# fatlipp/eacham

Measured on AMD Instinct MI355X. Metric: image-pairs matched/s + BA iters/s, 200-frame/50k-landmark synthetic, higher is better.
Workload: dtype i8; 1 GPU; S200 matching: 200 frames x 2000 kpts x 256-D, 19900 unordered pairs (both directions + mutual check); pairs_per_rank=19900, parallelism=pairs sharded over 1 GPU(s)

## Files before the change

eacham_amd/csrc/match_screen.hpp:

```cpp
#pragma once

#include <cmath>
#include <cstdint>

#if defined(__HIPCC__)
#define EACHAM_SCREEN_HD __host__ __device__
#else
#define EACHAM_SCREEN_HD
#endif

namespace eacham {
namespace screen {

constexpr int CENTRE = 64;
constexpr int STEP = 4;
constexpr int MAX_D2 = 256 * 255 * 255;
constexpr int MAX_M = 60;

EACHAM_SCREEN_HD inline int mag_value(int c) { return c < 16 ? c : (c < 24 ? 16 + 2 * (c - 16) : 32 + 4 * (c - 24)); }
EACHAM_SCREEN_HD inline int decode(int code) {
    const int m = mag_value(code & 31);
    return (code & 32) ? -m : m;
}
EACHAM_SCREEN_HD inline int encode(int x) {
    const int y = x - CENTRE;
    const int a = y < 0 ? -y : y;
    int c;
    if (a < 64) c = (a + 1) >> 2;
    else if (a < 128) c = 16 + ((a - 64 + 3) >> 3);
    else c = 24 + ((a - 128 + 7) >> 4);
    return (y < 0 && c != 0) ? (c | 32) : c;
}
EACHAM_SCREEN_HD inline int reconstruct(int code) { return CENTRE + STEP * decode(code); }

EACHAM_SCREEN_HD inline void pack32(const unsigned char* codes, uint32_t out[6]) {
    for (int w = 0; w < 6; ++w) out[w] = 0u;
    for (int e = 0; e < 32; ++e) {
        const int bit = 6 * e, w = bit >> 5, sh = bit & 31;
        const uint32_t v = codes[e] & 63u;
        out[w] |= v << sh;
        if (sh > 26) out[w + 1] |= v >> (32 - sh);
    }
}
EACHAM_SCREEN_HD inline int unpack32(const uint32_t in[6], int e) {
    const int bit = 6 * e, w = bit >> 5, sh = bit & 31;
    uint32_t v = in[w] >> sh;
    if (sh > 26) v |= in[w + 1] << (32 - sh);
    return (int)(v & 63u);
}

constexpr int STEP_BYTES = 1536, HI_PLANE = 1024, TILE_ROWS = 32;
struct FragSrc { int row, ks, h; };
EACHAM_SCREEN_HD constexpr FragSrc frag16_src(int u, int S, int lane) { return FragSrc{16 * u + (lane & 15), 2 * S + (lane >> 5), (lane >> 4) & 1}; }
EACHAM_SCREEN_HD constexpr int query16_tile(int s4) { return s4 >> 1; }
EACHAM_SCREEN_HD constexpr FragSrc query16_src(int s4, int S, int lane) { return frag16_src(s4 & 1, S, lane); }
EACHAM_SCREEN_HD constexpr int frag_lo_offset(FragSrc f) { return f.ks * STEP_BYTES + 16 * (f.row + TILE_ROWS * f.h); }
EACHAM_SCREEN_HD constexpr int frag_hi_offset(FragSrc f) { return f.ks * STEP_BYTES + HI_PLANE + 8 * (f.row + TILE_ROWS * f.h); }
EACHAM_SCREEN_HD constexpr int frag_kblock(FragSrc f) { return 2 * f.ks + f.h; }
EACHAM_SCREEN_HD constexpr int acc16_row(int u, int lane, int r) { return 16 * u + 4 * (lane >> 4) + r; }
EACHAM_SCREEN_HD constexpr bool frag16_separable() {
    for (int u = 0; u < 2; ++u)
        for (int S = 0; S < 2; ++S)
            for (int l = 0; l < 64; ++l) {
                if (frag_lo_offset(frag16_src(u, S, l)) != frag_lo_offset(frag16_src(0, 0, l)) + frag_lo_offset(frag16_src(u, S, 0))) return false;
                if (frag_hi_offset(frag16_src(u, S, l)) != frag_hi_offset(frag16_src(0, 0, l)) + frag_hi_offset(frag16_src(u, S, 0)) - HI_PLANE) return false;
            }
    return true;
}
static_assert(frag16_separable(), "lane offset + fragment offset");

EACHAM_SCREEN_HD inline double slack(int s_a, int e_b) { return sqrt((double)s_a) + sqrt((double)e_b); }

EACHAM_SCREEN_HD inline int lower_d2(unsigned n1, int s_a, int e_b) {
    const double l = (double)STEP * sqrt((double)n1) - slack(s_a, e_b);
    if (!(l > 0.0)) return 0;
    const double f = floor(l * l) - 1.0;
    return f <= 0.0 ? 0 : (f >= (double)MAX_D2 ? MAX_D2 : (int)f);
}
EACHAM_SCREEN_HD inline int upper_d2(unsigned u, int s_a, int e_b) {
    const double h = (double)STEP * sqrt((double)u) + slack(s_a, e_b);
    const double c = ceil(h * h) + 1.0;
    return c >= (double)MAX_D2 ? MAX_D2 : (int)c;
}

}
}
```

eacham_amd/csrc/matcher.hip:

```cpp
#include "context.hpp"
#include "match_plan.hpp"
#include "match_screen.hpp"
#include "match_tail.hpp"

#include <algorithm>
#include <climits>
#include <cstdlib>
#include <type_traits>

namespace eacham {

typedef int v4i __attribute__((ext_vector_type(4)));
typedef int v16i __attribute__((ext_vector_type(16)));
typedef const v4i __attribute__((address_space(1)))* gfrag_t;
typedef const int __attribute__((address_space(1)))* gint_t;

constexpr int PADH = 8350000;
constexpr int KEY_SHIFT = 7;
constexpr int KEY_MASK = (1 << KEY_SHIFT) - 1;
constexpr int CHUNK_TILES = 1 << KEY_SHIFT;
constexpr int MAX_ROWS = 16384;
constexpr int WG_THREADS = 256;
constexpr int WAVES = WG_THREADS / 64;
constexpr int MATCH_NSUB = 2;
// ... 690 lines not shown
    uint4* rr = rowres + (size_t)p * row_stride + ROWS_WAVE * wb;
#pragma unroll
    for (int s = 0; s < NSUB; ++s) {
        const int gi = ROWS_WAVE * wave + 32 * s + cl;
        const uint2 gc = GATHER ? pk[gi < item.y ? gi : 0] : make_uint2(0u, 0u);
        const int ca = GATHER ? ((gint_t)frames[pairs[gc.x].x].norm)[gc.y] : Aca[ROWS_WAVE * wb + 32 * s + cl];
        int cls1[2] = {e1[s], x1[s]}, cls2[2] = {e2[s], x2[s]}, clst[2] = {et[s], xt[s]};
        unsigned v1 = 0xffffffffu, v2 = 0xffffffffu, t1 = 0;
#pragma unroll
        for (int c = 0; c < 2; ++c) {
            const int o1 = __shfl_xor(cls1[c], 32), o2 = __shfl_xor(cls2[c], 32), ot = __shfl_xor(clst[c], 32);
            const int tt = o1 < cls1[c] ? ot : (o1 == cls1[c] ? imin(ot, clst[c]) : clst[c]);
            int m1 = cls1[c], m2 = cls2[c];
            top2_merge(m1, m2, o1, o2);
            const unsigned w1 = m1 == BIG ? 0xffffffffu : (unsigned)(2 * (m1 + ca) + c);
            const unsigned w2 = m2 == BIG ? 0xffffffffu : (unsigned)(2 * (m2 + ca) + c);
            t1 = w1 < v1 ? (unsigned)tt : t1;
            v2 = umin(umin(umax(v1, w1), v2), w2);
            v1 = umin(v1, w1);
        }
        if constexpr (GATHER) {
            if (h == 0 && gi < item.y) rowres[(size_t)gc.x * row_stride + gc.y] = make_uint4(v1, t1, v2, 0);
        } else {
            if (h == 0) rr[32 * s + cl] = make_uint4(v1, t1, v2, 0);
        }
    }
}

typedef int v2i __attribute__((ext_vector_type(2)));
typedef int v6i __attribute__((ext_vector_type(6)));
typedef int v8i __attribute__((ext_vector_type(8)));
typedef float v4f __attribute__((ext_vector_type(4)));
__device__ __forceinline__ void lds_read_frag64(v2i& dst, unsigned addr, int offset_bytes) {
    asm volatile("ds_read_b64 %0, %1 offset:%2" : "=v"(dst) : "v"(addr), "n"(offset_bytes));
}
__device__ __forceinline__ float fmin3(float a, float b, float c) {
    float d;
    asm("v_min3_f32 %0, %1, %2, %3" : "=v"(d) : "v"(a), "v"(b), "v"(c));
    return d;
}
template <int METRIC>
__device__ __forceinline__ bool ratio_pass(int d2_best, int d2_second, double ratio);
struct OpenList {
    const int* seghead;
    int* segcount;
    uint2* cands;
    int2* items;
    int* n_items;
};
struct ScreenFrag { v4i lo; v2i hi; };
__device__ __forceinline__ v8i screen_operand(const ScreenFrag& f) { return v8i{f.lo[0], f.lo[1], f.lo[2], f.lo[3], f.hi[0], f.hi[1], 0, 0}; }

template <int METRIC>
__global__ __launch_bounds__(WG_THREADS, 3) void match_screen_kernel(const FrameDev* __restrict__ frames, const int2* __restrict__ pairs,
                                                                     int wgs_per_pair, uint4* __restrict__ rowres, int row_stride, double ratio,
                                                                     unsigned long long* __restrict__ openmask, int mask_stride,
                                                                     OpenList ol) {
    constexpr int NSUB = 2;
    constexpr int NQ = 4, NU = 2, NS = 2;
    constexpr int KS = NU * NS;
    static_assert(KS == SCREEN_KS && 2 * NS == SCREEN_KS && screen::STEP_BYTES == SCREEN_STEP_BYTES, "match_screen.hpp maps this stored tile");
    constexpr int TILE_V4 = SCREEN_TILE_BYTES / 16;
    constexpr int ROWS_WAVE = 32 * NSUB, ROWS_WG = WAVES * ROWS_WAVE;
    constexpr float BIGF = 3.0e38f;
    constexpr int SCALE = (int)0x82828282u;
    constexpr int NT = SCREEN_CALL_TILES, RING = 3 * NT;
    static_assert(NT == 2 && KS == 4 && NT * 32 == 64, "the waits of a call are counted for two tiles of four steps; wave 0 carries the constants of a call");
    __shared__ v4i sB[RING][TILE_V4];
    __shared__ __attribute__((aligned(16))) float sHb[RING][32];
    const int tid = threadIdx.x;
    const int lane = tid & 63;
    const int wave = __builtin_amdgcn_readfirstlane(tid >> 6);
    const int rb = blockIdx.x % wgs_per_pair;
    const int p = blockIdx.x / wgs_per_pair;
    const int2 pr = pairs[p];
    const FrameDev A = frames[pr.x], B = frames[pr.y];
    const int A_even = ((gint_t)A.meta)[0], A_tiles = ((gint_t)A.meta)[1];
    const int T = ((gint_t)B.meta)[2];
    if (rb * (ROWS_WG / 32) >= A_tiles) return;
    const int wb = rb * WAVES + wave;
    const bool active = NSUB * wb < A_tiles;
    typedef const __attribute__((address_space(1))) char* gbytes_t;
    typedef const float __attribute__((address_space(1)))* gfloat_t;
    const gbytes_t Aimg = (gbytes_t)A.screen, Bimg = (gbytes_t)B.screen;
    const gfloat_t Am2 = (gfloat_t)(Aimg + (size_t)A.ntiles * SCREEN_TILE_BYTES), Bm2 = (gfloat_t)(Bimg + (size_t)B.ntiles * SCREEN_TILE_BYTES);
    const int wbc = active ? wb : 0;

    v6i a[NQ][NS];
#pragma unroll
    for (int s = 0; s < NQ; ++s)
#pragma unroll
        for (int S = 0; S < NS; ++S) {
            const screen::FragSrc src = screen::query16_src(s, S, lane);
            const gbytes_t tb = Aimg + (size_t)(NSUB * wbc + screen::query16_tile(s)) * SCREEN_TILE_BYTES;
            const v4i lo = *(const v4i __attribute__((address_space(1)))*)(tb + screen::frag_lo_offset(src));
            const v2i hi = *(const v2i __attribute__((address_space(1)))*)(tb + screen::frag_hi_offset(src));
            a[s][S] = v6i{lo[0] ^ 0x20820820, lo[1] ^ 0x08208208, lo[2] ^ (int)0x82082082u, lo[3] ^ 0x20820820, hi[0] ^ 0x08208208, hi[1] ^ (int)0x82082082u};
        }
    float xm[2][NQ][NU];
#pragma unroll
    for (int q = 0; q < 2; ++q)
#pragma unroll
        for (int s = 0; s < NQ; ++s)
#pragma unroll
            for (int u = 0; u < NU; ++u) xm[q][s][u] = BIGF;

    static_assert(TILE_V4 % 64 == 0, "a tile is a whole number of 1 KiB pieces");
    constexpr int PIECES = TILE_V4 / 64;
    static_assert((NT * PIECES) % WAVES == 0, "every wave stages the same number of pieces per call");
    constexpr int PPW = NT * PIECES / WAVES;
    const int TM = T - 1;
    unsigned stage_off = (unsigned)lane * 16u, hb_off = (unsigned)(lane & 31) * 4u;
    auto stage_piece = [&](int tile, int slot, int piece) {
        const gbytes_t base = Bimg + (size_t)min(tile, TM) * SCREEN_TILE_BYTES + piece * 1024;
        asm volatile("" : "+v"(stage_off));
        __builtin_amdgcn_global_load_lds((const __attribute__((address_space(1))) void*)(base + stage_off),
                                         (__attribute__((address_space(3))) void*)(&sB[slot][piece * 64]), 16, 0, 0);
    };
    auto load_hb = [&](int tile) {
        asm volatile("" : "+v"(hb_off));
        const gbytes_t row = reinterpret_cast<gbytes_t>(Bm2) + (size_t)128 * min(tile + (lane >> 5), TM);
        return *reinterpret_cast<gfloat_t>(row + hb_off);
    };
    const int t0 = T > 0 && !(T & 1) ? 1 : 0;
    float hb_new = 0.0f;
    if (T > 0) {
#pragma unroll
        for (int i = 0; i < ((2 * NT + 2) * PIECES + WAVES - 1) / WAVES; ++i) {
            const int idx = wave + WAVES * i, v = idx / PIECES;
            if (v < 2 * NT + 1 + t0) stage_piece(v, v < t0 ? RING - 1 : v - t0, idx % PIECES);
        }
        if (tid < 32 * (NT + 2 + t0)) {
            const int v = tid >> 5;
            sHb[v < t0 ? RING - 1 : v - t0][tid & 31] = Bm2[32 * min(v, TM) + (tid & 31)];
        }
        if (wave == 0) hb_new = load_hb(NT + 2 + t0);
    }
    __builtin_amdgcn_s_waitcnt(0);
    __syncthreads();

    typedef const v4f __attribute__((address_space(3)))* lds_v4f_t;
    lds_v4f_t hb_lane = (lds_v4f_t)(const __attribute__((address_space(3))) void*)&sHb[0][screen::acc16_row(0, lane, 0)];
    asm volatile("" : "+v"(hb_lane));
    auto cinit_of = [&](int slot, int u) { return hb_lane[8 * slot + 4 * u]; };
    int scale = SCALE;
    asm volatile("" : "+v"(scale));
    auto mfma = [&](const ScreenFrag& b, const v6i& q, const v4f& c) {
        const v8i q8 = __builtin_shufflevector(q, q, 0, 1, 2, 3, 4, 5, -1, -1);
        return __builtin_amdgcn_mfma_scale_f32_16x16x128_f8f6f4(screen_operand(b), q8, c, 2, 2, 0, scale, 0, scale);
    };
    v4f accA[NU][NQ], accB[NU][NQ];
#pragma unroll
    for (int u = 0; u < NU; ++u)
#pragma unroll
        for (int s = 0; s < NQ; ++s) accA[u][s] = v4f{0.0f, 0.0f, 0.0f, 0.0f}, accB[u][s] = v4f{0.0f, 0.0f, 0.0f, 0.0f};
    ScreenFrag bq[3];
    const char* sBb = reinterpret_cast<const char*>(&sB[0][0]);
    auto tile_plain = [&](int slot) {
#pragma unroll
        for (int S = 0; S < NS; ++S)
#pragma unroll
            for (int u = 0; u < NU; ++u) {
                const screen::FragSrc src = screen::frag16_src(u, S, lane);
                ScreenFrag f;
                f.lo = *reinterpret_cast<const v4i*>(sBb + slot * SCREEN_TILE_BYTES + screen::frag_lo_offset(src));
                f.hi = *reinterpret_cast<const v2i*>(sBb + slot * SCREEN_TILE_BYTES + screen::frag_hi_offset(src));
                const v4f c0 = cinit_of(slot, u);
#pragma unroll
                for (int s = 0; s < NQ; ++s) accA[u][s] = mfma(f, a[s][S], S ? accA[u][s] : c0);
            }
    };
#pragma unroll
    for (int i = 0; i < 3; ++i) bq[i].lo = v4i{0, 0, 0, 0}, bq[i].hi = v2i{0, 0};
    unsigned lds16 = lds_addr(sBb) + (unsigned)screen::frag_lo_offset(screen::frag16_src(0, 0, lane));
    unsigned lds8 = lds_addr(sBb) + (unsigned)(screen::frag_hi_offset(screen::frag16_src(0, 0, lane)) - screen::HI_PLANE);
    asm volatile("" : "+v"(lds16), "+v"(lds8));
    auto frag_lo_imm = [](int slot, int f) constexpr { return slot * SCREEN_TILE_BYTES + screen::frag_lo_offset(screen::frag16_src(f % NU, f / NU, 0)); };
    auto frag_hi_imm = [](int slot, int f) constexpr { return slot * SCREEN_TILE_BYTES + screen::frag_hi_offset(screen::frag16_src(f % NU, f / NU, 0)); };
    unsigned hb_rd = lds_addr(&sHb[0][screen::acc16_row(0, lane, 0)]), hb_wr = lds_addr(&sHb[0][0]) + 4u * lane;
    asm volatile("" : "+v"(hb_rd), "+v"(hb_wr));
    v4f ci[NU];
#pragma unroll
    for (int u = 0; u < NU; ++u) ci[u] = v4f{0.0f, 0.0f, 0.0f, 0.0f};
    auto cinit_issue = [&](int slot) {
#pragma unroll
        for (int u = 0; u < NU; ++u) lds_read_frag(ci[u], hb_rd, 128 * slot + 64 * u);
    };
    auto drain_lds = [&]() {
        asm volatile("s_waitcnt lgkmcnt(0)"
                     : "+v"(bq[0].lo), "+v"(bq[0].hi), "+v"(bq[1].lo), "+v"(bq[1].hi), "+v"(bq[2].lo), "+v"(bq[2].hi), "+v"(ci[0]), "+v"(ci[1]));
    };
    if (T > 0 && active) {
        if (t0) {
            tile_plain(RING - 1);
#pragma unroll
            for (int s = 0; s < NQ; ++s)
#pragma unroll
                for (int u = 0; u < NU; ++u) xm[1][s][u] = fminf(fminf(accA[u][s][0], accA[u][s][1]), fminf(accA[u][s][2], accA[u][s][3]));
        }
        tile_plain(0);
        cinit_issue(1);
#pragma unroll
        for (int f = 0; f < 2; ++f) {
            lds_read_frag(bq[f].lo, lds16, frag_lo_imm(1, f));
            lds_read_frag64(bq[f].hi, lds8, frag_hi_imm(1, f));
        }
        drain_lds();
    }
    __syncthreads();
    auto key_lo = [](int ks) constexpr { return ks >= KS - 1 ? 32 : (32 * ks + KS - 2) / (KS - 1); };
    auto consume = [&](const v4f(&cur)[NU][NQ], float(&m)[NQ][NU], const int idx) {
        const int u = idx / (4 * NQ), s = (idx / 4) % NQ, eg = idx % 4;
        if (eg & 1) m[s][u] = fmin3(m[s][u], cur[u][s][eg - 1], cur[u][s][eg]);
    };
    auto call = [&](auto K3c, const int t) {
        constexpr int K3 = decltype(K3c)::value;
        constexpr int BASE = NT * K3;
        constexpr int PH = (K3 * ((NT * KS) % 3)) % 3;
        auto stage = [&](int i) {
            const int idx = wave + WAVES * i, later = idx >= PIECES ? 1 : 0;
            stage_piece(t + 2 * NT + 1 + later, later ? (BASE + 2 * NT + 2) % RING : (BASE + 2 * NT + 1) % RING, idx - PIECES * later);
        };
        if (wave == 0) {
            asm volatile("ds_write_b32 %0, %1 offset:%2" : : "v"(hb_wr), "v"(hb_new), "n"(((BASE + NT + 2) % RING) * 128) : "memory");
            hb_new = load_hb(t + 2 * NT + 2);
        }
        auto half = [&](auto HHc) {
            constexpr int HH = decltype(HHc)::value;
            v4f(&cur)[NU][NQ] = HH ? accB : accA;
            v4f(&nxt)[NU][NQ] = HH ? accA : accB;
#pragma unroll
            for (int ks = 0; ks < KS; ++ks) {
                const int i = HH * KS + ks, j = i + 2;
                ScreenFrag& f = bq[(i + PH) % 3];
                const int u = ks % NU, S = ks / NU;
                if (ks == 0) {
                    asm volatile("s_waitcnt lgkmcnt(2)" : "+v"(f.lo), "+v"(f.hi), "+v"(ci[0]), "+v"(ci[1]));
                } else if (ks < KS - 1) {
                    asm volatile("s_waitcnt lgkmcnt(2)" : "+v"(f.lo), "+v"(f.hi));
                } else {
                    asm volatile("s_waitcnt lgkmcnt(4)" : "+v"(f.lo), "+v"(f.hi));
                }
                lds_read_frag(bq[(j + PH) % 3].lo, lds16, frag_lo_imm((BASE + 1 + j / KS) % RING, j % KS));
                lds_read_frag64(bq[(j + PH) % 3].hi, lds8, frag_hi_imm((BASE + 1 + j / KS) % RING, j % KS));
#pragma unroll
                for (int s = 0; s < NQ; ++s) nxt[u][s] = mfma(f, a[s][S], S ? nxt[u][s] : ci[u]);
#pragma unroll
                for (int idx = key_lo(ks); idx < key_lo(ks + 1); ++idx) {
                    consume(cur, xm[HH], idx);
                    if (idx == 31) cinit_issue((BASE + HH + 2) % RING);
                }
                if (i % 2 == 0 && i / 2 < PPW) stage(i / 2);
                __builtin_amdgcn_sched_barrier(0);
            }
        };
        if (active) {
            half(std::integral_constant<int, 0>{});
            half(std::integral_constant<int, 1>{});
        } else {
#pragma unroll
            for (int i = 0; i < PPW; ++i) stage(i);
        }
        asm volatile("s_waitcnt vmcnt(1)" : : : "memory");
        __builtin_amdgcn_s_barrier();
    };
    auto last = [&]() {
        if (active) {
#pragma unroll
            for (int s = 0; s < NQ; ++s)
#pragma unroll
                for (int u = 0; u < NU; ++u)
                    xm[0][s][u] = fminf(xm[0][s][u], fminf(fminf(accA[u][s][0], accA[u][s][1]), fminf(accA[u][s][2], accA[u][s][3])));
        }
    };
    if (T > 0) {
        const int NC = (TM - t0) / 2;
        int c = 0;
        for (; c + 3 <= NC; c += 3) {
            call(std::integral_constant<int, 0>{}, t0 + NT * c);
            call(std::integral_constant<int, 1>{}, t0 + NT * (c + 1));
            call(std::integral_constant<int, 2>{}, t0 + NT * (c + 2));
        }
        if (c < NC) call(std::integral_constant<int, 0>{}, t0 + NT * c);
        if (c + 1 < NC) call(std::integral_constant<int, 1>{}, t0 + NT * (c + 1));
        asm volatile("s_waitcnt vmcnt(0)" : : : "memory");
        drain_lds();
        last();
    }
    if (!active) return;
    const gint_t Asr = (gint_t)(Am2 + 32 * (size_t)A.ntiles);
    const int e_b = T > 0 ? ((gint_t)(Bm2 + 64 * (size_t)B.ntiles))[0] : 0;
    uint4* rr = rowres + (size_t)p * row_stride + ROWS_WAVE * wb;
    const int lane_t = (int)((hb_wr - lds_addr(&sHb[0][0])) >> 2);
    constexpr unsigned PAD_V = 2u * PADH;
    float v1 = BIGF, v2 = BIGF;
#pragma unroll
    for (int s = 0; s < NQ; ++s) {
        float m1 = BIGF, m2 = BIGF;
#pragma unroll
        for (int q = 0; q < 2; ++q)
#pragma unroll
            for (int u = 0; u < NU; ++u) {
                const float mine = xm[q][s][u];
                m2 = fminf(m2, fmaxf(m1, mine)), m1 = fminf(m1, mine);
            }
#pragma unroll
        for (int x = 16; x <= 32; x *= 2) {
            const float o1 = __shfl_xor(m1, x), o2 = __shfl_xor(m2, x);
            m2 = fminf(fmaxf(m1, o1), fminf(m2, o2)), m1 = fminf(m1, o1);
        }
        if ((lane_t >> 4) == s) v1 = m1, v2 = m2;
    }
    unsigned long long open_rows = 0;
    {
        const int s = lane_t >> 5;
        const int j = ROWS_WAVE * wb + lane_t;
        const float ma = Am2[j];
        const bool real_row = ma < 0.5f * SCREEN_PAD;
        const bool real1 = real_row && v1 < 0.5f * SCREEN_PAD, real2 = real_row && v2 < 0.5f * SCREEN_PAD;
        const unsigned pa = NSUB * wb + s >= A_even ? 1u : 0u;
        const int s_a = Asr[j];
        const unsigned n1 = real1 ? (unsigned)(2.0f * (v1 + ma)) : 0u, u = real2 ? (unsigned)(2.0f * (v2 + ma)) : 0u;
        const unsigned w1 = real1 ? (unsigned)screen::lower_d2(n1, s_a, e_b) - pa + 2u : 0xffffffffu;
        const unsigned w2 = real2 ? (unsigned)screen::upper_d2(u, s_a, e_b) - pa + 2u : 0xffffffffu;
        rr[lane_t] = make_uint4(w1, 0u, w2, real1 ? n1 : 0xffffffffu);
        const bool open = NSUB * wb + s < A_tiles && w1 < PAD_V && (w2 >= PAD_V || ratio_pass<METRIC>((int)(w1 + pa) - 2, (int)(w2 + pa) - 2, ratio));
        open_rows = __ballot(open);
    }
    if (!openmask) return;
    if (lane_t == 0) openmask[(size_t)p * mask_stride + wb] = open_rows;
    const int c = __popcll(open_rows);
    if (c == 0) return;
    const int head = ol.seghead[p];
    int pos = 0;
    if (lane_t == 0) pos = atomicAdd(&ol.segcount[head], c);
    pos = __shfl(pos, 0);
    if ((open_rows >> lane_t) & 1)
        ol.cands[(size_t)head * row_stride + pos + __popcll(open_rows & ((1ull << lane_t) - 1))] = make_uint2((unsigned)p, (unsigned)(ROWS_WAVE * wb + lane_t));
    const int k = (pos + GATHER_WIDTH - 1) / GATHER_WIDTH;
    if (lane_t == 0 && GATHER_WIDTH * k < pos + c) ol.items[atomicAdd(ol.n_items, 1)] = make_int2(head, k);
}


constexpr int METRIC_L2 = 0, METRIC_HAMMING = 1;
template <int METRIC>
__device__ __forceinline__ bool ratio_pass(int d2_best, int d2_second, double ratio) {
    if (METRIC == METRIC_HAMMING) return d2_best >= 0 && d2_second >= 0 && (double)__fdiv_rn((float)d2_best, (float)d2_second) < ratio;
    float q = __fdiv_rn(__fsqrt_rn((float)d2_best), __fsqrt_rn((float)d2_second));
    return (double)q < ratio;
}

template <int METRIC>
__global__ __launch_bounds__(FIN_THREADS) void match_finalize_kernel(
    const FrameDev* __restrict__ frames, const int2* __restrict__ pairs,
    const uint4* __restrict__ rowres, const uint2* __restrict__ colpart, int col_chunks, int wb_stride,
    int row_stride, double ratio, int min_dir, int min_mutual, int mode,
    uint2* __restrict__ out_matches, int* __restrict__ counts, int4* __restrict__ stats) {
    extern __shared__ int smem[];
    const int tid = threadIdx.x;
    const int p = blockIdx.x;
    const int2 pr = pairs[p];
    const FrameDev A = frames[pr.x], B = frames[pr.y];
    const int A_even = A.meta[0], A_tiles = A.meta[1], B_even = B.meta[0], B_tiles = B.meta[1];
    int* keepcol = smem;
    int* bwd = smem + row_stride;
    __shared__ int s_cnt[3];
    if (tid < 3) s_cnt[tid] = 0;
    __syncthreads();
    constexpr unsigned PAD_V = 2u * PADH;

    int c12 = 0, c21 = 0;
    constexpr int WG_TILES = ROWS_PER_WG / 32;
    const int nslots = (A_tiles + WG_TILES - 1) / WG_TILES + 1;
    const int first_odd = A_even / WG_TILES + 1;
    for (int c = tid; c < 32 * B_tiles; c += FIN_THREADS) {
        int d = -1;
        if (B.orig[c] >= 0) {
            unsigned v1 = 0xffffffffu, v2 = 0xffffffffu;
            const uint2* cp = colpart + (size_t)p * wb_stride * row_stride + c;
            for (int k = 0; k < nslots; ++k) {
                const bool even = WG_TILES * k < A_even;
                if (!even && k < first_odd) continue;
                const uint2 e = cp[(size_t)k * row_stride];
                const unsigned pa = even ? 0u : 1u;
                const unsigned va = ((e.x >> (KEY_SHIFT + 1)) << 1) | pa, vb = ((e.y >> (KEY_SHIFT + 1)) << 1) | pa;
                v2 = umin(umin(umax(v1, va), v2), vb);
                v1 = umin(v1, va);
            }
            const unsigned pb = (c >> 5) >= B_even ? 1u : 0u;
            const bool ok = v2 < PAD_V && ratio_pass<METRIC>((int)(v1 + pb) - 2, (int)(v2 + pb) - 2, ratio);
            d = ok ? (int)(v1 + pb) - 2 : -1;
            c21 += ok;
        }
// ... 610 lines not shown
            EACHAM_HIP_TRY(ctx, hipGetLastError());
        }
    }
    commit_frame(ctx, f, kind, n, dim, ks, ntiles, 0);
    return EACHAM_OK;
}

static int check_integer_flag(eacham_ctx* ctx) {
    if (ctx->kind_common == FRAME_F32) return EACHAM_OK;
    int flag = 0;
    EACHAM_HIP_TRY(ctx, hipMemcpyAsync(&flag, &ctx->flag_dev->not_integer, sizeof(int), hipMemcpyDeviceToHost, ctx->stream));
    EACHAM_HIP_TRY(ctx, hipStreamSynchronize(ctx->stream));
    if (flag) {
        EACHAM_HIP_TRY(ctx, hipMemsetAsync(&ctx->flag_dev->not_integer, 0, sizeof(int), ctx->stream));
        return ctx->fail(EACHAM_ERR_NOT_INTEGER,
                         "descriptors must be integer-valued in [0,255] for the exact int8 path");
    }
    return EACHAM_OK;
}

static unsigned long long* colprune_totals(eacham_ctx* ctx) { return ctx->flag_dev->colprune; }
static unsigned long long* screen_tally(eacham_ctx* ctx) { return ctx->flag_dev->screen; }
static bool frames_have_screen(const eacham_ctx* ctx) {
    if (ctx->kind_common == FRAME_F32 || ctx->ks_common != SCREEN_EXACT_KS) return false;
    for (const auto& f : ctx->frames)
        if (f.n > 0 && !f.screen) return false;
    return true;
}

static MatchPlan make_plan(const eacham_ctx* ctx, int npairs, bool full_cols) {
    int max_tiles = std::max(4, GROUP_TILES);
    for (const auto& f : ctx->frames)
        if (f.n >= 0) max_tiles = std::max(max_tiles, f.tiles_used);
    return make_plan(MatchPlanIn{max_tiles, npairs, (size_t)ctx->match_budget_mb << 20, full_cols, ctx->match_no_overlap});
}

struct MatchCall {
    eacham_ctx* ctx;
    MatchPlan pl;
    CallArrays call;
    hipStream_t st1, st2;
    double ratio;
    int min_dir, min_mutual, mode;
    size_t fin_smem;
    bool screen_sweep, bound_sweep;
};
struct MatchLaunch {
    Slot s;
    const int2* pb;
    int nb, first, b;
    int* cnt;
};

template <int METRIC>
static void launch_sweep(const MatchCall& c, const MatchLaunch& l) {
    const MatchPlan& pl = c.pl;
    const FrameDev* frames = c.ctx->frame_table_dev;
    with_ks(c.ctx->ks_common, [&](auto ks) {
        constexpr int KS = decltype(ks)::value;
        if (c.screen_sweep)
            match_screen_kernel<METRIC><<<l.nb * pl.wgs_per_pair, WG_THREADS, 0, c.st1>>>(
                frames, l.pb, pl.wgs_per_pair, l.s.rowres, pl.row_stride, c.ratio, l.s.openmask, pl.mask_stride,
                OpenList{c.call.seghead + l.first, c.call.segcount + l.first, l.s.rowcand, l.s.items, c.call.launch_items + l.b});
        else if (pl.full_cols)
            match_tile_kernel<KS><<<l.nb * pl.wgs_per_pair * pl.col_chunks, WG_THREADS, 0, c.st1>>>(
                frames, l.pb, pl.wgs_per_pair, pl.col_chunks, l.s.rowres, l.s.colpart, pl.wb_stride, pl.row_stride);
        else if (c.bound_sweep)
            match_sweep_kernel<KS, true><<<l.nb * pl.wgs_per_pair, WG_THREADS, 0, c.st1>>>(frames, l.pb, pl.wgs_per_pair, l.s.rowres, pl.row_stride);
        else
            match_sweep_kernel<KS, false><<<l.nb * pl.wgs_per_pair, WG_THREADS, 0, c.st1>>>(frames, l.pb, pl.wgs_per_pair, l.s.rowres, pl.row_stride);
    });
}

static void launch_open_rows_exact(const MatchCall& c, const MatchLaunch& l) {
    const int ggrid = l.nb * ((c.pl.row_stride + GATHER_WIDTH - 1) / GATHER_WIDTH + 1);
    match_sweep_kernel<SCREEN_EXACT_KS, false, true><<<ggrid, WG_THREADS, 0, c.st1>>>(
        c.ctx->frame_table_dev, l.pb, 0, l.s.rowres, c.pl.row_stride,
        GatherList<true>{l.s.rowcand, c.call.segcount + l.first, l.s.items, c.call.launch_items + l.b});
}

template <int METRIC>
static void launch_full_cols_tail(const MatchCall& c, const MatchLaunch& l, int4* stats) {
    match_finalize_kernel<METRIC><<<l.nb, FIN_THREADS, c.fin_smem, c.st2>>>(c.ctx->frame_table_dev, l.pb, l.s.rowres, l.s.colpart, c.pl.col_chunks, c.pl.wb_stride,
                                                                     c.pl.row_stride, c.ratio, c.min_dir, c.min_mutual, c.mode, l.s.matches, l.cnt, stats);
}

template <int METRIC>
static int launch_lean_tail(const MatchCall& c, const MatchLaunch& l) {
    eacham_ctx* ctx = c.ctx;
    const MatchPlan& pl = c.pl;
    const Slot& s = l.s;
    const FrameDev* frames = ctx->frame_table_dev;
    hipStream_t st2 = c.st2;
    const int nb = l.nb, mode = c.mode;
    int *n_items = &s.counters->n_items, *n_pre = &s.counters->n_pre, *n_aitems = &s.counters->n_aitems;
    const int vgrid = std::min(std::max(nb * pl.wgs_per_pair, 1), 512);
    const int agrid = std::min(std::max(nb * pl.wgs_per_pair, 1), 4096);
    EACHAM_HIP_TRY(ctx, hipMemsetAsync(s.counters, 0, sizeof(SlotCounters), st2));
    if (c.screen_sweep)
        match_opentally_kernel<<<(nb + TALLY_THREADS - 1) / TALLY_THREADS, TALLY_THREADS, 0, st2>>>(c.call.seghead + l.first, c.call.segcount + l.first, nb,
                                                                                               c.call.launch_items + l.b, screen_tally(ctx));
    with_ks(ctx->ks_common, [&](auto ks) {
        constexpr int KS = decltype(ks)::value;
        if (c.bound_sweep) {
            match_rowpick_kernel<METRIC><<<nb, FIN_THREADS, 0, st2>>>(frames, l.pb, s.rowres, pl.row_stride, c.ratio, s.candlist, s.state, s.items, n_pre);
            match_colverify_kernel<KS, true><<<vgrid, WG_THREADS, 0, st2>>>(frames, l.pb, nullptr, s.candlist, s.state, s.items, n_pre, pl.row_stride, 0, nullptr, s.rowres);
        }
        if (METRIC == METRIC_L2 && c.screen_sweep && mode == 0)
            match_rows2_kernel<METRIC_L2, true><<<nb, FIN_THREADS, 0, st2>>>(frames, l.pb, s.rowres, pl.row_stride, c.ratio, c.min_dir, c.min_mutual, mode, s.rowcand,
                                                                      s.candlist, s.bytile, s.state, s.aitems, n_aitems, s.openmask, pl.mask_stride);
        else
            match_rows2_kernel<METRIC><<<nb, FIN_THREADS, 0, st2>>>(frames, l.pb, s.rowres, pl.row_stride, c.ratio, c.min_dir, c.min_mutual, mode, s.rowcand,
                                                            s.candlist, s.bytile, s.state, s.aitems, n_aitems);
        match_argmin_kernel<KS, METRIC><<<agrid, 64, 0, st2>>>(frames, l.pb, s.rowcand, s.bytile, s.aitems, n_aitems, pl.row_stride, mode == 0 ? s.colres : nullptr,
                                                       s.state, c.ratio, ctx->match_colprune ? 1 : 0);
// ... 330 lines not shown
    *settled = (int64_t)tot[0];
    *verified = (int64_t)tot[1];
    return EACHAM_OK;
}

int eacham_match_debug_screen(eacham_ctx* ctx, int64_t* rows, int64_t* open) {
    if (!ctx) return EACHAM_ERR_INVALID;
    std::lock_guard<std::mutex> lock(ctx->mu);
    (void)hipSetDevice(ctx->device);
    if (!rows || !open) return ctx->fail(EACHAM_ERR_INVALID, "null output");
    unsigned long long tot[2] = {0, 0};
    EACHAM_HIP_TRY(ctx, hipStreamSynchronize(ctx->stream));
    EACHAM_HIP_TRY(ctx, hipMemcpy(tot, screen_tally(ctx), sizeof(tot), hipMemcpyDeviceToHost));
    *rows = (int64_t)tot[0];
    *open = (int64_t)tot[1];
    return EACHAM_OK;
}

int eacham_match_debug_screen_items(eacham_ctx* ctx, int64_t* items) {
    if (!ctx) return EACHAM_ERR_INVALID;
    std::lock_guard<std::mutex> lock(ctx->mu);
    (void)hipSetDevice(ctx->device);
    if (!items) return ctx->fail(EACHAM_ERR_INVALID, "null output");
    unsigned long long n = 0;
    EACHAM_HIP_TRY(ctx, hipStreamSynchronize(ctx->stream));
    EACHAM_HIP_TRY(ctx, hipMemcpy(&n, screen_tally(ctx) + 2, sizeof(n), hipMemcpyDeviceToHost));
    *items = (int64_t)n;
    return EACHAM_OK;
}

int eacham_match_debug_screen_pair(eacham_ctx* ctx, int f1, int f2, uint32_t* n1, int32_t* l1, int32_t* u2, int cap) {
    return match_entry(ctx, [&]() -> int {
        if (!n1 || !l1 || !u2 || cap < 0) return ctx->fail(EACHAM_ERR_INVALID, "null output");
        const int32_t pr[2] = {f1, f2};
        int rc = check_pairs_host(ctx, pr, 1);
        if (rc) return rc;
        rc = check_integer_flag(ctx);
        if (rc) return rc;
        rc = sync_frame_table(ctx);
        if (rc) return rc;
        if (!frames_have_screen(ctx)) return ctx->fail(EACHAM_ERR_UNSUPPORTED, "the screen sweep needs int8 frames above 128-D");
        const FrameHost& A = ctx->frames[f1];
        if (cap < A.n) return ctx->fail(EACHAM_ERR_CAPACITY, "%d rows but capacity %d", A.n, cap);
        if (A.n == 0) return EACHAM_OK;
        const MatchPlan pl = make_plan(ctx, 1, false);
        rc = ensure_workspace(ctx, pl.total);
        if (rc) return rc;
        uint4* const rowres = pl.slot(ctx->ws, 0).rowres;
        IoStage io(ctx, ctx->stream);
        const auto h_pair = io.in<int2>(pr, 1);
        IoDev d;
        rc = io.upload(d);
        if (rc) return rc;
        match_screen_kernel<METRIC_L2><<<pl.wgs_per_pair, WG_THREADS, 0, ctx->stream>>>(ctx->frame_table_dev, d(h_pair), pl.wgs_per_pair, rowres, pl.row_stride, 0.0, nullptr, 0,
                                                                                        OpenList{});
        EACHAM_HIP_TRY(ctx, hipGetLastError());
        rc = io.finish();
        if (rc) return rc;
        const int rows = 32 * A.tiles_used;
        std::vector<uint4> res((size_t)rows);
        std::vector<int> pos((size_t)A.n), meta(2);
        EACHAM_HIP_TRY(ctx, hipMemcpy(res.data(), rowres, sizeof(uint4) * res.size(), hipMemcpyDeviceToHost));
        EACHAM_HIP_TRY(ctx, hipMemcpy(pos.data(), A.pos, sizeof(int) * pos.size(), hipMemcpyDeviceToHost));
        EACHAM_HIP_TRY(ctx, hipMemcpy(meta.data(), A.meta, sizeof(int) * 2, hipMemcpyDeviceToHost));
        for (int q = 0; q < A.n; ++q) {
            const int j = pos[q];
            const uint4 e = res[j];
            const unsigned pa = (j >> 5) >= meta[0] ? 1u : 0u;
            n1[q] = e.w;
            l1[q] = e.x == 0xffffffffu ? -1 : (int32_t)(e.x + pa) - 2;
            u2[q] = e.z == 0xffffffffu ? -1 : (int32_t)(e.z + pa) - 2;
        }
        return EACHAM_OK;
    });
}

int eacham_match_pairs_directed(eacham_ctx* ctx, const int32_t* pairs, int npairs, double ratio, int32_t* counts,
                                int64_t* offsets, uint32_t* out_q, uint32_t* out_t, int64_t cap, int64_t* out_total) {
    return match_entry(ctx, [&]() -> int {
        return match_pairs_host(ctx, MATCH_L2, pairs, npairs, ratio, 0, 0, 1, counts, offsets, out_q, out_t, nullptr, cap, out_total, nullptr);
    });
}

int eacham_match_pair_dot(eacham_ctx* ctx, int f1, int f2, float min_score, uint32_t* out_q, uint32_t* out_t, float* out_score,
                          int cap, int* out_count) {
    return match_entry(ctx, [&]() -> int {
        if (!out_count) return ctx->fail(EACHAM_ERR_INVALID, "null output");
        const int32_t pr[2] = {f1, f2};
        int32_t count = 0;
        int64_t offsets[2] = {0, 0}, total = 0;
        const int rc = match_pairs_host(ctx, MATCH_DOT, pr, 1, min_score, 0, 0, 1, &count, offsets, out_q, out_t, out_score, cap, &total, nullptr);
        if (rc == EACHAM_OK || rc == EACHAM_ERR_CAPACITY) *out_count = (int)total;
        return rc;
    });
}

int eacham_match_pairs_directed_dot(eacham_ctx* ctx, const int32_t* pairs, int npairs, float min_score, int32_t* counts,
                                    int64_t* offsets, uint32_t* out_q, uint32_t* out_t, float* out_score, int64_t cap,
                                    int64_t* out_total) {
    return match_entry(ctx, [&]() -> int {
        return match_pairs_host(ctx, MATCH_DOT, pairs, npairs, min_score, 0, 0, 1, counts, offsets, out_q, out_t, out_score, cap, out_total, nullptr);
    });
}

int eacham_match_all_pairs_dot(eacham_ctx* ctx, const int32_t* pairs, int npairs, float min_score, int min_dir, int min_mutual,
                               int32_t* counts, int64_t* offsets, uint32_t* out_q, uint32_t* out_t, float* out_score, int64_t cap,
                               int64_t* out_total, int32_t* stats) {
// ... 139 lines not shown
```

Before: 2.066 million image-pairs/s.

## Double query sub-tiles per wave in screen kernel to reuse train fragments

Each wave in the screen sweep now holds eight query sub-tiles (two wave-blocks of 64 rows) instead of four, so every train fragment read from LDS feeds twice as many MFMAs. The ping-pong accumulators are merged into one set, and the min-reduction is interleaved into the MFMA groups. The grid is halved to match, and launch bounds drop to two WGs per SIMD because register use rises. This trades occupancy and grid parallelism for less LDS traffic per MFMA. It also risks tail imbalance and register spills.

Result: faster. 2.154 million image-pairs/s (median of 6 runs) (+4.3%).

```diff
diff --git a/eacham_amd/csrc/match_screen.hpp b/eacham_amd/csrc/match_screen.hpp
--- a/eacham_amd/csrc/match_screen.hpp
+++ b/eacham_amd/csrc/match_screen.hpp
@@ -54,6 +54,22 @@
 EACHAM_SCREEN_HD constexpr FragSrc frag16_src(int u, int S, int lane) { return FragSrc{16 * u + (lane & 15), 2 * S + (lane >> 5), (lane >> 4) & 1}; }
 EACHAM_SCREEN_HD constexpr int query16_tile(int s4) { return s4 >> 1; }
 EACHAM_SCREEN_HD constexpr FragSrc query16_src(int s4, int S, int lane) { return frag16_src(s4 & 1, S, lane); }
+constexpr int QUERY_SUBTILES = 8;
+EACHAM_SCREEN_HD constexpr int query16_block(int s8) { return s8 >> 2; }
+EACHAM_SCREEN_HD constexpr int query16_wave_row(int s8, int lane) { return TILE_ROWS * query16_tile(s8) + query16_src(s8, 0, lane).row; }
+constexpr bool query16_eight() {
+    for (int s8 = 0; s8 < QUERY_SUBTILES; ++s8)
+        for (int l = 0; l < 64; ++l) {
+            if (query16_tile(s8) != 2 * query16_block(s8) + query16_tile(s8 & 3) || query16_tile(s8) >= QUERY_SUBTILES / 2) return false;
+            if (query16_wave_row(s8, l) != 16 * s8 + (l & 15)) return false;
+            for (int S = 0; S < 2; ++S) {
+                const FragSrc f = query16_src(s8, S, l), g = query16_src(s8 & 3, S, l), t = frag16_src(0, S, l);
+                if (f.row != g.row || f.ks != g.ks || f.h != g.h || f.ks != t.ks || f.h != t.h) return false;
+            }
+        }
+    return true;
+}
+static_assert(query16_eight(), "eight sub-tiles = two wave-blocks of the four-sub-tile map, the train side's K blocks");
 EACHAM_SCREEN_HD constexpr int frag_lo_offset(FragSrc f) { return f.ks * STEP_BYTES + 16 * (f.row + TILE_ROWS * f.h); }
 EACHAM_SCREEN_HD constexpr int frag_hi_offset(FragSrc f) { return f.ks * STEP_BYTES + HI_PLANE + 8 * (f.row + TILE_ROWS * f.h); }
 EACHAM_SCREEN_HD constexpr int frag_kblock(FragSrc f) { return 2 * f.ks + f.h; }
diff --git a/eacham_amd/csrc/matcher.hip b/eacham_amd/csrc/matcher.hip
--- a/eacham_amd/csrc/matcher.hip
+++ b/eacham_amd/csrc/matcher.hip
@@ -766,12 +766,14 @@
 __device__ __forceinline__ v8i screen_operand(const ScreenFrag& f) { return v8i{f.lo[0], f.lo[1], f.lo[2], f.lo[3], f.hi[0], f.hi[1], 0, 0}; }
 
 template <int METRIC>
-__global__ __launch_bounds__(WG_THREADS, 3) void match_screen_kernel(const FrameDev* __restrict__ frames, const int2* __restrict__ pairs,
+__global__ __launch_bounds__(WG_THREADS, 2) void match_screen_kernel(const FrameDev* __restrict__ frames, const int2* __restrict__ pairs,
                                                                      int wgs_per_pair, uint4* __restrict__ rowres, int row_stride, double ratio,
                                                                      unsigned long long* __restrict__ openmask, int mask_stride,
                                                                      OpenList ol) {
-    constexpr int NSUB = 2;
-    constexpr int NQ = 4, NU = 2, NS = 2;
+    constexpr int WBS = 2, WB_TILES = 2;
+    constexpr int NSUB = WBS * WB_TILES;
+    constexpr int NQ = screen::QUERY_SUBTILES, NU = 2, NS = 2;
+    static_assert(NQ == 2 * NSUB && screen::query16_block(NQ - 1) == WBS - 1, "match_screen.hpp maps the wave's eight sub-tiles");
     constexpr int KS = NU * NS;
     static_assert(KS == SCREEN_KS && 2 * NS == SCREEN_KS && screen::STEP_BYTES == SCREEN_STEP_BYTES, "match_screen.hpp maps this stored tile");
     constexpr int TILE_V4 = SCREEN_TILE_BYTES / 16;
@@ -792,13 +794,12 @@
     const int A_even = ((gint_t)A.meta)[0], A_tiles = ((gint_t)A.meta)[1];
     const int T = ((gint_t)B.meta)[2];
     if (rb * (ROWS_WG / 32) >= A_tiles) return;
-    const int wb = rb * WAVES + wave;
-    const bool active = NSUB * wb < A_tiles;
+    const int wv = rb * WAVES + wave;
+    const bool active = NSUB * wv < A_tiles;
     typedef const __attribute__((address_space(1))) char* gbytes_t;
     typedef const float __attribute__((address_space(1)))* gfloat_t;
     const gbytes_t Aimg = (gbytes_t)A.screen, Bimg = (gbytes_t)B.screen;
     const gfloat_t Am2 = (gfloat_t)(Aimg + (size_t)A.ntiles * SCREEN_TILE_BYTES), Bm2 = (gfloat_t)(Bimg + (size_t)B.ntiles * SCREEN_TILE_BYTES);
-    const int wbc = active ? wb : 0;
 
     v6i a[NQ][NS];
 #pragma unroll
@@ -806,7 +807,8 @@
 #pragma unroll
         for (int S = 0; S < NS; ++S) {
             const screen::FragSrc src = screen::query16_src(s, S, lane);
-            const gbytes_t tb = Aimg + (size_t)(NSUB * wbc + screen::query16_tile(s)) * SCREEN_TILE_BYTES;
+            const int qt = NSUB * wv + screen::query16_tile(s);
+            const gbytes_t tb = Aimg + (size_t)(qt < A_tiles ? qt : 0) * SCREEN_TILE_BYTES;
             const v4i lo = *(const v4i __attribute__((address_space(1)))*)(tb + screen::frag_lo_offset(src));
             const v2i hi = *(const v2i __attribute__((address_space(1)))*)(tb + screen::frag_hi_offset(src));
             a[s][S] = v6i{lo[0] ^ 0x20820820, lo[1] ^ 0x08208208, lo[2] ^ (int)0x82082082u, lo[3] ^ 0x20820820, hi[0] ^ 0x08208208, hi[1] ^ (int)0x82082082u};
@@ -833,7 +835,7 @@
     };
     auto load_hb = [&](int tile) {
         asm volatile("" : "+v"(hb_off));
-        const gbytes_t row = reinterpret_cast<gbytes_t>(Bm2) + (size_t)128 * min(tile + (lane >> 5), TM);
+        const gbytes_t row = reinterpret_cast<gbytes_t>(Bm2) + (size_t)128 * min(tile + (int)(stage_off >> 9), TM);
         return *reinterpret_cast<gfloat_t>(row + hb_off);
     };
     const int t0 = T > 0 && !(T & 1) ? 1 : 0;
@@ -863,11 +865,11 @@
         const v8i q8 = __builtin_shufflevector(q, q, 0, 1, 2, 3, 4, 5, -1, -1);
         return __builtin_amdgcn_mfma_scale_f32_16x16x128_f8f6f4(screen_operand(b), q8, c, 2, 2, 0, scale, 0, scale);
     };
-    v4f accA[NU][NQ], accB[NU][NQ];
+    v4f acc[NU][NQ];
 #pragma unroll
     for (int u = 0; u < NU; ++u)
 #pragma unroll
-        for (int s = 0; s < NQ; ++s) accA[u][s] = v4f{0.0f, 0.0f, 0.0f, 0.0f}, accB[u][s] = v4f{0.0f, 0.0f, 0.0f, 0.0f};
+        for (int s = 0; s < NQ; ++s) acc[u][s] = v4f{0.0f, 0.0f, 0.0f, 0.0f};
     ScreenFrag bq[3];
     const char* sBb = reinterpret_cast<const char*>(&sB[0][0]);
     auto tile_plain = [&](int slot) {
@@ -881,8 +883,12 @@
                 f.hi = *reinterpret_cast<const v2i*>(sBb + slot * SCREEN_TILE_BYTES + screen::frag_hi_offset(src));
                 const v4f c0 = cinit_of(slot, u);
 #pragma unroll
-                for (int s = 0; s < NQ; ++s) accA[u][s] = mfma(f, a[s][S], S ? accA[u][s] : c0);
+                for (int s = 0; s < NQ; ++s) acc[u][s] = mfma(f, a[s][S], S ? acc[u][s] : c0);
             }
+    };
+    auto consume_plain = [&](float(&m)[NQ][NU], int u) {
+#pragma unroll
+        for (int s = 0; s < NQ; ++s) m[s][u] = fminf(m[s][u], fminf(fminf(acc[u][s][0], acc[u][s][1]), fminf(acc[u][s][2], acc[u][s][3])));
     };
 #pragma unroll
     for (int i = 0; i < 3; ++i) bq[i].lo = v4i{0, 0, 0, 0}, bq[i].hi = v2i{0, 0};
@@ -907,12 +913,10 @@
     if (T > 0 && active) {
         if (t0) {
             tile_plain(RING - 1);
-#pragma unroll
-            for (int s = 0; s < NQ; ++s)
-#pragma unroll
-                for (int u = 0; u < NU; ++u) xm[1][s][u] = fminf(fminf(accA[u][s][0], accA[u][s][1]), fminf(accA[u][s][2], accA[u][s][3]));
+            consume_plain(xm[1], 0), consume_plain(xm[1], 1);
         }
         tile_plain(0);
+        consume_plain(xm[0], 0);
         cinit_issue(1);
 #pragma unroll
         for (int f = 0; f < 2; ++f) {
@@ -922,10 +926,9 @@
         drain_lds();
     }
     __syncthreads();
-    auto key_lo = [](int ks) constexpr { return ks >= KS - 1 ? 32 : (32 * ks + KS - 2) / (KS - 1); };
-    auto consume = [&](const v4f(&cur)[NU][NQ], float(&m)[NQ][NU], const int idx) {
-        const int u = idx / (4 * NQ), s = (idx / 4) % NQ, eg = idx % 4;
-        if (eg & 1) m[s][u] = fmin3(m[s][u], cur[u][s][eg - 1], cur[u][s][eg]);
+    auto consume = [&](float(&m)[NQ][NU], const int u, const int s) {
+        m[s][u] = fmin3(m[s][u], acc[u][s][0], acc[u][s][1]);
+        m[s][u] = fmin3(m[s][u], acc[u][s][2], acc[u][s][3]);
     };
     auto call = [&](auto K3c, const int t) {
         constexpr int K3 = decltype(K3c)::value;
@@ -941,8 +944,6 @@
         }
         auto half = [&](auto HHc) {
             constexpr int HH = decltype(HHc)::value;
-            v4f(&cur)[NU][NQ] = HH ? accB : accA;
-            v4f(&nxt)[NU][NQ] = HH ? accA : accB;
 #pragma unroll
             for (int ks = 0; ks < KS; ++ks) {
                 const int i = HH * KS + ks, j = i + 2;
@@ -958,12 +959,17 @@
                 lds_read_frag(bq[(j + PH) % 3].lo, lds16, frag_lo_imm((BASE + 1 + j / KS) % RING, j % KS));
                 lds_read_frag64(bq[(j + PH) % 3].hi, lds8, frag_hi_imm((BASE + 1 + j / KS) % RING, j % KS));
 #pragma unroll
-                for (int s = 0; s < NQ; ++s) nxt[u][s] = mfma(f, a[s][S], S ? nxt[u][s] : ci[u]);
-#pragma unroll
-                for (int idx = key_lo(ks); idx < key_lo(ks + 1); ++idx) {
-                    consume(cur, xm[HH], idx);
-                    if (idx == 31) cinit_issue((BASE + HH + 2) % RING);
+                for (int g = 0; g < NQ / 2; ++g) {
+#pragma unroll
+                    for (int s = 2 * g; s < 2 * g + 2; ++s) acc[u][s] = mfma(f, a[s][S], S ? acc[u][s] : ci[u]);
+#pragma unroll
+                    for (int s = 2 * g; s < 2 * g + 2; ++s) {
+                        if (ks == 0) consume(xm[HH], 1, s);
+                        if (ks == KS - 1) consume(xm[1 - HH], 0, s);
+                    }
+                    if (g < NQ / 2 - 1) __builtin_amdgcn_sched_barrier(0);
                 }
+                if (ks == 2) cinit_issue((BASE + HH + 2) % RING);
                 if (i % 2 == 0 && i / 2 < PPW) stage(i / 2);
                 __builtin_amdgcn_sched_barrier(0);
             }
@@ -979,13 +985,7 @@
         __builtin_amdgcn_s_barrier();
     };
     auto last = [&]() {
-        if (active) {
-#pragma unroll
-            for (int s = 0; s < NQ; ++s)
-#pragma unroll
-                for (int u = 0; u < NU; ++u)
-                    xm[0][s][u] = fminf(xm[0][s][u], fminf(fminf(accA[u][s][0], accA[u][s][1]), fminf(accA[u][s][2], accA[u][s][3])));
-        }
+        if (active) consume_plain(xm[0], 1);
     };
     if (T > 0) {
         const int NC = (TM - t0) / 2;
@@ -1002,57 +1002,66 @@
         last();
     }
     if (!active) return;
+    constexpr int ROWS_WB = 32 * WB_TILES;
     const gint_t Asr = (gint_t)(Am2 + 32 * (size_t)A.ntiles);
     const int e_b = T > 0 ? ((gint_t)(Bm2 + 64 * (size_t)B.ntiles))[0] : 0;
-    uint4* rr = rowres + (size_t)p * row_stride + ROWS_WAVE * wb;
     const int lane_t = (int)((hb_wr - lds_addr(&sHb[0][0])) >> 2);
     constexpr unsigned PAD_V = 2u * PADH;
-    float v1 = BIGF, v2 = BIGF;
-#pragma unroll
-    for (int s = 0; s < NQ; ++s) {
-        float m1 = BIGF, m2 = BIGF;
-#pragma unroll
-        for (int q = 0; q < 2; ++q)
-#pragma unroll
-            for (int u = 0; u < NU; ++u) {
-                const float mine = xm[q][s][u];
-                m2 = fminf(m2, fmaxf(m1, mine)), m1 = fminf(m1, mine);
+    auto tail = [&](auto Hc) {
+        constexpr int H = decltype(Hc)::value;
+        const int wb = WBS * wv + H;
+        if (WB_TILES * wb >= A_tiles) return;
+        uint4* rr = rowres + (size_t)p * row_stride + ROWS_WB * wb;
+        float v1 = BIGF, v2 = BIGF;
+#pragma unroll
+        for (int s = 0; s < NQ / WBS; ++s) {
+            static_assert(screen::query16_block(NQ / WBS * H) == H, "the sub-tiles of wave-block H");
+            float m1 = BIGF, m2 = BIGF;
+#pragma unroll
+            for (int q = 0; q < 2; ++q)
+#pragma unroll
+                for (int u = 0; u < NU; ++u) {
+                    const float mine = xm[q][NQ / WBS * H + s][u];
+                    m2 = fminf(m2, fmaxf(m1, mine)), m1 = fminf(m1, mine);
+                }
+#pragma unroll
+            for (int x = 16; x <= 32; x *= 2) {
+                const float o1 = __shfl_xor(m1, x), o2 = __shfl_xor(m2, x);
+                m2 = fminf(fmaxf(m1, o1), fminf(m2, o2)), m1 = fminf(m1, o1);
             }
-#pragma unroll
-        for (int x = 16; x <= 32; x *= 2) {
-            const float o1 = __shfl_xor(m1, x), o2 = __shfl_xor(m2, x);
-            m2 = fminf(fmaxf(m1, o1), fminf(m2, o2)), m1 = fminf(m1, o1);
-        }
-        if ((lane_t >> 4) == s) v1 = m1, v2 = m2;
-    }
-    unsigned long long open_rows = 0;
-    {
-        const int s = lane_t >> 5;
-        const int j = ROWS_WAVE * wb + lane_t;
-        const float ma = Am2[j];
-        const bool real_row = ma < 0.5f * SCREEN_PAD;
-        const bool real1 = real_row && v1 < 0.5f * SCREEN_PAD, real2 = real_row && v2 < 0.5f * SCREEN_PAD;
-        const unsigned pa = NSUB * wb + s >= A_even ? 1u : 0u;
-        const int s_a = Asr[j];
-        const unsigned n1 = real1 ? (unsigned)(2.0f * (v1 + ma)) : 0u, u = real2 ? (unsigned)(2.0f * (v2 + ma)) : 0u;
-        const unsigned w1 = real1 ? (unsigned)screen::lower_d2(n1, s_a, e_b) - pa + 2u : 0xffffffffu;
-        const unsigned w2 = real2 ? (unsigned)screen::upper_d2(u, s_a, e_b) - pa + 2u : 0xffffffffu;
-        rr[lane_t] = make_uint4(w1, 0u, w2, real1 ? n1 : 0xffffffffu);
-        const bool open = NSUB * wb + s < A_tiles && w1 < PAD_V && (w2 >= PAD_V || ratio_pass<METRIC>((int)(w1 + pa) - 2, (int)(w2 + pa) - 2, ratio));
-        open_rows = __ballot(open);
-    }
-    if (!openmask) return;
-    if (lane_t == 0) openmask[(size_t)p * mask_stride + wb] = open_rows;
-    const int c = __popcll(open_rows);
-    if (c == 0) return;
-    const int head = ol.seghead[p];
-    int pos = 0;
-    if (lane_t == 0) pos = atomicAdd(&ol.segcount[head], c);
-    pos = __shfl(pos, 0);
-    if ((open_rows >> lane_t) & 1)
-        ol.cands[(size_t)head * row_stride + pos + __popcll(open_rows & ((1ull << lane_t) - 1))] = make_uint2((unsigned)p, (unsigned)(ROWS_WAVE * wb + lane_t));
-    const int k = (pos + GATHER_WIDTH - 1) / GATHER_WIDTH;
-    if (lane_t == 0 && GATHER_WIDTH * k < pos + c) ol.items[atomicAdd(ol.n_items, 1)] = make_int2(head, k);
+            if ((lane_t >> 4) == s) v1 = m1, v2 = m2;
+        }
+        unsigned long long open_rows = 0;
+        {
+            const int s = lane_t >> 5;
+            const int j = ROWS_WB * wb + lane_t;
+            const float ma = Am2[j];
+            const bool real_row = ma < 0.5f * SCREEN_PAD;
+            const bool real1 = real_row && v1 < 0.5f * SCREEN_PAD, real2 = real_row && v2 < 0.5f * SCREEN_PAD;
+            const unsigned pa = WB_TILES * wb + s >= A_even ? 1u : 0u;
+            const int s_a = Asr[j];
+            const unsigned n1 = real1 ? (unsigned)(2.0f * (v1 + ma)) : 0u, u = real2 ? (unsigned)(2.0f * (v2 + ma)) : 0u;
+            const unsigned w1 = real1 ? (unsigned)screen::lower_d2(n1, s_a, e_b) - pa + 2u : 0xffffffffu;
+            const unsigned w2 = real2 ? (unsigned)screen::upper_d2(u, s_a, e_b) - pa + 2u : 0xffffffffu;
+            rr[lane_t] = make_uint4(w1, 0u, w2, real1 ? n1 : 0xffffffffu);
+            const bool open = WB_TILES * wb + s < A_tiles && w1 < PAD_V && (w2 >= PAD_V || ratio_pass<METRIC>((int)(w1 + pa) - 2, (int)(w2 + pa) - 2, ratio));
+            open_rows = __ballot(open);
+        }
+        if (!openmask) return;
+        if (lane_t == 0) openmask[(size_t)p * mask_stride + wb] = open_rows;
+        const int c = __popcll(open_rows);
+        if (c == 0) return;
+        const int head = ol.seghead[p];
+        int pos = 0;
+        if (lane_t == 0) pos = atomicAdd(&ol.segcount[head], c);
+        pos = __shfl(pos, 0);
+        if ((open_rows >> lane_t) & 1)
+            ol.cands[(size_t)head * row_stride + pos + __popcll(open_rows & ((1ull << lane_t) - 1))] = make_uint2((unsigned)p, (unsigned)(ROWS_WB * wb + lane_t));
+        const int k = (pos + GATHER_WIDTH - 1) / GATHER_WIDTH;
+        if (lane_t == 0 && GATHER_WIDTH * k < pos + c) ol.items[atomicAdd(ol.n_items, 1)] = make_int2(head, k);
+    };
+    tail(std::integral_constant<int, 0>{});
+    tail(std::integral_constant<int, 1>{});
 }
 
 
@@ -1769,6 +1778,7 @@
     int* cnt;
 };
 
+static int screen_wgs_per_pair(const MatchPlan& pl) { return (pl.wgs_per_pair + 1) / 2; }
 template <int METRIC>
 static void launch_sweep(const MatchCall& c, const MatchLaunch& l) {
     const MatchPlan& pl = c.pl;
@@ -1776,8 +1786,8 @@
     with_ks(c.ctx->ks_common, [&](auto ks) {
         constexpr int KS = decltype(ks)::value;
         if (c.screen_sweep)
-            match_screen_kernel<METRIC><<<l.nb * pl.wgs_per_pair, WG_THREADS, 0, c.st1>>>(
-                frames, l.pb, pl.wgs_per_pair, l.s.rowres, pl.row_stride, c.ratio, l.s.openmask, pl.mask_stride,
+            match_screen_kernel<METRIC><<<l.nb * screen_wgs_per_pair(pl), WG_THREADS, 0, c.st1>>>(
+                frames, l.pb, screen_wgs_per_pair(pl), l.s.rowres, pl.row_stride, c.ratio, l.s.openmask, pl.mask_stride,
                 OpenList{c.call.seghead + l.first, c.call.segcount + l.first, l.s.rowcand, l.s.items, c.call.launch_items + l.b});
         else if (pl.full_cols)
             match_tile_kernel<KS><<<l.nb * pl.wgs_per_pair * pl.col_chunks, WG_THREADS, 0, c.st1>>>(
@@ -2214,7 +2224,7 @@
         IoDev d;
         rc = io.upload(d);
         if (rc) return rc;
-        match_screen_kernel<METRIC_L2><<<pl.wgs_per_pair, WG_THREADS, 0, ctx->stream>>>(ctx->frame_table_dev, d(h_pair), pl.wgs_per_pair, rowres, pl.row_stride, 0.0, nullptr, 0,
+        match_screen_kernel<METRIC_L2><<<screen_wgs_per_pair(pl), WG_THREADS, 0, ctx->stream>>>(ctx->frame_table_dev, d(h_pair), screen_wgs_per_pair(pl), rowres, pl.row_stride, 0.0, nullptr, 0,
                                                                                         OpenList{});
         EACHAM_HIP_TRY(ctx, hipGetLastError());
         rc = io.finish();
```
